# AliBahri94/GM3D

Measured on AMD Instinct MI355X. Metric: point-clouds/sec pretrain step (N=1024,G=64), higher is better.
Workload: dtype bf16

## Files before the change

gm3d_amd/csrc/embed.hip:

```cpp
#include "common.hpp"
#include "guided.hpp"

namespace gm3d {


__device__ __forceinline__ int tpr_of(int C) { return C >> 3; }

__global__ __launch_bounds__(256) void moments3_kernel(const float* __restrict__ x, int R, double* __restrict__ partial) {
    __shared__ double red[4][9];
    double s[9];
#pragma unroll
    for (int i = 0; i < 9; ++i) s[i] = 0.0;
    for (int r = blockIdx.x * 256 + threadIdx.x; r < R; r += gridDim.x * 256) {
        const double a = x[(size_t)r * 3], b = x[(size_t)r * 3 + 1], c = x[(size_t)r * 3 + 2];
        s[0] += a; s[1] += b; s[2] += c;
        s[3] += a * a; s[4] += a * b; s[5] += a * c; s[6] += b * b; s[7] += b * c; s[8] += c * c;
    }
#pragma unroll
    for (int i = 0; i < 9; ++i) {
        double v = s[i];
        for (int o = 32; o > 0; o >>= 1) v += __shfl_xor(v, o);
        if ((threadIdx.x & 63) == 0) red[threadIdx.x >> 6][i] = v;
    }
    __syncthreads();
    if (threadIdx.x < 9) partial[(size_t)blockIdx.x * 9 + threadIdx.x] =
        (red[0][threadIdx.x] + red[1][threadIdx.x]) + (red[2][threadIdx.x] + red[3][threadIdx.x]);
}

template <class T>
__global__ __launch_bounds__(256) void pn_layer1_fwd_kernel(const float* __restrict__ x, const float* __restrict__ wf,
                                                            const float* __restrict__ bf, T* __restrict__ a1, int R, int C1) {
    const int tpr = C1 >> 3;
    const size_t total = (size_t)R * tpr;
    for (size_t t = (size_t)blockIdx.x * 256 + threadIdx.x; t < total; t += (size_t)gridDim.x * 256) {
        const size_t r = t / tpr;
        const int c = (int)(t - r * tpr) * 8;
        const float a = x[r * 3], b = x[r * 3 + 1], d = x[r * 3 + 2];
        float v[8];
#pragma unroll
        for (int i = 0; i < 8; ++i) {
            const float h = a * wf[(c + i) * 3] + b * wf[(c + i) * 3 + 1] + d * wf[(c + i) * 3 + 2] + bf[c + i];
            v[i] = h > 0.f ? h : 0.f;
        }
        V8<T>::store(a1 + r * C1 + c, v);
    }
}

template <class T>
__global__ __launch_bounds__(256) void group_max_fwd_kernel(const T* __restrict__ in, const float* __restrict__ bias,
                                                            T* __restrict__ out, uint8_t* __restrict__ arg, int G, int K, int C) {
    const int tpr = C >> 3, gpb = blockDim.x / tpr;
    const int lane = threadIdx.x % tpr, gl = threadIdx.x / tpr, c = lane * 8;
    for (int g = blockIdx.x * gpb + gl; g < G; g += gridDim.x * gpb) {
        const T* base = in + (size_t)g * K * C + c;
        float best[8];
        int bk[8];
#pragma unroll
        for (int i = 0; i < 8; ++i) { best[i] = -INFINITY; bk[i] = 0; }
        int k = 0;
        for (; k + 8 <= K; k += 8) {
            float v[8][8];
#pragma unroll
            for (int u = 0; u < 8; ++u) V8<T>::load(base + (size_t)(k + u) * C, v[u]);
#pragma unroll
            for (int u = 0; u < 8; ++u)
#pragma unroll
                for (int i = 0; i < 8; ++i)
                    if (v[u][i] > best[i]) { best[i] = v[u][i]; bk[i] = k + u; }
        }
        for (; k < K; ++k) {
            float v[8];
            V8<T>::load(base + (size_t)k * C, v);
#pragma unroll
            for (int i = 0; i < 8; ++i)
                if (v[i] > best[i]) { best[i] = v[i]; bk[i] = k; }
        }
#pragma unroll
        for (int i = 0; i < 8; ++i) {
            if (bias) best[i] += bias[c + i];
            arg[(size_t)g * C + c + i] = (uint8_t)bk[i];
        }
        V8<T>::store(out + (size_t)g * C + c, best);
    }
}

template <class T>
__global__ __launch_bounds__(256) void group_max_bwd_kernel(const T* __restrict__ dout, const uint8_t* __restrict__ arg, T* __restrict__ din,
                                     int G, int K, int C) {
    const int tpr = C >> 3, SL = blockDim.x / tpr;
    const int lane = threadIdx.x % tpr, sl = threadIdx.x / tpr, c = lane * 8;
    for (int g = blockIdx.x; g < G; g += gridDim.x) {
        float d[8];
        V8<T>::load(dout + (size_t)g * C + c, d);
        int a[8];
#pragma unroll
        for (int i = 0; i < 8; ++i) a[i] = arg[(size_t)g * C + c + i];
        for (int k = sl; k < K; k += SL) {
            float v[8];
#pragma unroll
            for (int i = 0; i < 8; ++i) v[i] = a[i] == k ? d[i] : 0.f;
            V8<T>::store(din + ((size_t)g * K + k) * C + c, v);
        }
    }
}

template <int NQ>
__device__ __forceinline__ void write_partials(float (&acc)[NQ][8], float* sm, float* partial, int C, int c, int sl, int SL) {
#pragma unroll
    for (int q = 0; q < NQ; ++q)
#pragma unroll
        for (int i = 0; i < 8; ++i) sm[(size_t)sl * NQ * C + q * C + c + i] = acc[q][i];
    __syncthreads();
    for (int t = threadIdx.x; t < NQ * C; t += blockDim.x) {
        float s = 0.f;
        for (int s2 = 0; s2 < SL; ++s2) s += sm[(size_t)s2 * NQ * C + t];
        partial[(size_t)blockIdx.x * NQ * C + t] = s;
    }
}

template <class T>
__global__ __launch_bounds__(256) void bn_bcast_stats_kernel(const T* __restrict__ y0, const T* __restrict__ t, int G, int K, int C,
                                      float* __restrict__ partial) {
    extern __shared__ float sm[];
    const int tpr = C >> 3, SL = blockDim.x / tpr;
    const int lane = threadIdx.x % tpr, sl = threadIdx.x / tpr, c = lane * 8;
    float acc[2][8];
#pragma unroll
    for (int i = 0; i < 8; ++i) acc[0][i] = acc[1][i] = 0.f;
    for (int g = blockIdx.x; g < G; g += gridDim.x) {
        float tv[8];
        V8<T>::load(t + (size_t)g * C + c, tv);
        for (int k = sl; k < K; k += SL) {
            float v[8];
            V8<T>::load(y0 + ((size_t)g * K + k) * C + c, v);
#pragma unroll
            for (int i = 0; i < 8; ++i) { const float y = v[i] + tv[i]; acc[0][i] += y; acc[1][i] += y * y; }
        }
    }
    write_partials<2>(acc, sm, partial, C, c, sl, SL);
}

template <class T>
__global__ __launch_bounds__(256) void bn_bcast_apply_relu_kernel(const T* __restrict__ y0, const T* __restrict__ t, const float* __restrict__ scale,
                                           const float* __restrict__ shift, T* __restrict__ a2, int G, int K, int C,
                                           float slope, const int* __restrict__ sel ) {
    const int tpr = C >> 3, SL = blockDim.x / tpr;
    const int lane = threadIdx.x % tpr, sl = threadIdx.x / tpr, c = lane * 8;
    float sc[8], sh[8];
#pragma unroll
    for (int i = 0; i < 8; ++i) { sc[i] = scale[c + i]; sh[i] = shift[c + i]; }
    for (int g = blockIdx.x; g < G; g += gridDim.x) {
        const int sg = sel ? sel[g] : g;
        float tv[8];
        V8<T>::load(t + (size_t)sg * C + c, tv);
        for (int k = sl; k < K; k += SL) {
            float v[8];
            V8<T>::load(y0 + ((size_t)sg * K + k) * C + c, v);
#pragma unroll
            for (int i = 0; i < 8; ++i) { const float h = (v[i] + tv[i]) * sc[i] + sh[i]; v[i] = h > 0.f ? h : slope * h; }
            V8<T>::store(a2 + ((size_t)g * K + k) * C + c, v);
        }
    }
}

template <class T>
__global__ __launch_bounds__(256) void bn_bcast_bwd_stats_kernel(const T* __restrict__ da2, const T* __restrict__ y0, const T* __restrict__ t,
                                          const float* __restrict__ scale, const float* __restrict__ shift,
                                          const float* __restrict__ mean, const float* __restrict__ rstd, int G, int K, int C,
                                          float* __restrict__ partial, float slope,
                                          const int* __restrict__ sel ) {
    extern __shared__ float sm[];
    const int tpr = C >> 3, SL = blockDim.x / tpr;
    const int lane = threadIdx.x % tpr, sl = threadIdx.x / tpr, c = lane * 8;
    float sc[8], sh[8], mu[8], rs[8], acc[2][8];
#pragma unroll
    for (int i = 0; i < 8; ++i) { sc[i] = scale[c + i]; sh[i] = shift[c + i]; mu[i] = mean[c + i]; rs[i] = rstd[c + i]; acc[0][i] = acc[1][i] = 0.f; }
    for (int g = blockIdx.x; g < G; g += gridDim.x) {
        const int sg = sel ? sel[g] : g;
        float tv[8];
        V8<T>::load(t + (size_t)sg * C + c, tv);
        for (int k = sl; k < K; k += SL) {
            float v[8], d[8];
            V8<T>::load(y0 + ((size_t)sg * K + k) * C + c, v);
            V8<T>::load(da2 + ((size_t)g * K + k) * C + c, d);
// ... 25 lines not shown
        sc[i] = scale[c + i]; sh[i] = shift[c + i]; mu[i] = mean[c + i]; rs[i] = rstd[c + i];
        m1[i] = s1[c + i] * inv_rows; m2[i] = s2[c + i] * inv_rows;
    }
    for (int g = blockIdx.x * gpb + gl; g < G; g += gridDim.x * gpb) {
        const int cg = inv ? inv[g] : g;
        float tv[8], gs[8];
        V8<T>::load(t + (size_t)g * C + c, tv);
#pragma unroll
        for (int i = 0; i < 8; ++i) gs[i] = 0.f;
        int k = 0;
        for (; k + 4 <= K; k += 4) {
            float v[4][8], d[4][8];
#pragma unroll
            for (int u = 0; u < 4; ++u) {
                V8<T>::load(y0 + ((size_t)g * K + k + u) * C + c, v[u]);
                if (cg >= 0) V8<T>::load(da2 + ((size_t)cg * K + k + u) * C + c, d[u]);
                else {
#pragma unroll
                    for (int i = 0; i < 8; ++i) d[u][i] = 0.f;
                }
            }
#pragma unroll
            for (int u = 0; u < 4; ++u) {
#pragma unroll
                for (int i = 0; i < 8; ++i) {
                    const float y = v[u][i] + tv[i];
                    const float gg = (y * sc[i] + sh[i] > 0.f) ? d[u][i] : slope * d[u][i];
                    const float r = sc[i] * (gg - m1[i] - (y - mu[i]) * rs[i] * m2[i]);
                    v[u][i] = r; gs[i] += r;
                }
                V8<T>::store(dy + ((size_t)g * K + k + u) * C + c, v[u]);
            }
        }
        for (; k < K; ++k) {
            float v[8], d[8] = {0.f, 0.f, 0.f, 0.f, 0.f, 0.f, 0.f, 0.f};
            const size_t o = ((size_t)g * K + k) * C + c;
            V8<T>::load(y0 + o, v);
            if (cg >= 0) V8<T>::load(da2 + ((size_t)cg * K + k) * C + c, d);
#pragma unroll
            for (int i = 0; i < 8; ++i) {
                const float y = v[i] + tv[i];
                const float gg = (y * sc[i] + sh[i] > 0.f) ? d[i] : slope * d[i];
                const float r = sc[i] * (gg - m1[i] - (y - mu[i]) * rs[i] * m2[i]);
                v[i] = r; gs[i] += r;
            }
            V8<T>::store(dy + o, v);
        }
#pragma unroll
        for (int i = 0; i < 8; ++i) dt[(size_t)g * C + c + i] = gs[i];
    }
}

template <class T>
__global__ __launch_bounds__(256) void group_scatter_add_kernel(T* __restrict__ df, const T* __restrict__ dfg, const uint8_t* __restrict__ arg,
                                         int G, int K, int C, float* __restrict__ partial) {
    extern __shared__ float sm[];
    const int tpr = C >> 3, SL = blockDim.x / tpr;
    const int lane = threadIdx.x % tpr, sl = threadIdx.x / tpr, c = lane * 8;
    float acc[1][8];
#pragma unroll
    for (int i = 0; i < 8; ++i) acc[0][i] = 0.f;
    for (int g = blockIdx.x; g < G; g += gridDim.x) {
        float d[8];
        int a[8];
        V8<T>::load(dfg + (size_t)g * C + c, d);
#pragma unroll
        for (int i = 0; i < 8; ++i) a[i] = arg[(size_t)g * C + c + i];
        for (int k = sl; k < K; k += SL) {
            float v[8];
            const size_t o = ((size_t)g * K + k) * C + c;
            V8<T>::load(df + o, v);
            bool hit = false;
#pragma unroll
            for (int i = 0; i < 8; ++i) {
                if (a[i] == k) { v[i] += d[i]; hit = true; }
                acc[0][i] += v[i];
            }
            if (hit) V8<T>::store(df + o, v);
        }
    }
    write_partials<1>(acc, sm, partial, C, c, sl, SL);
}

template <class T>
__global__ __launch_bounds__(256) void pn_layer1_bwd_stats_kernel(const T* __restrict__ da1, const T* __restrict__ a1, const float* __restrict__ x,
                                           const float* __restrict__ w1, const float* __restrict__ b1,
                                           const float* __restrict__ mean, const float* __restrict__ rstd,
                                           const float* __restrict__ xmean, int R, int C1, double* __restrict__ partial) {
    extern __shared__ double smd[];
    const int tpr = C1 >> 3, SL = blockDim.x / tpr;
    const int lane = threadIdx.x % tpr, sl = threadIdx.x / tpr, c = lane * 8;
    float wx[8], wy[8], wz[8], bb[8], rs[8];
    double acc[5][8];
    const float mx = xmean[0], my = xmean[1], mz = xmean[2];
#pragma unroll
    for (int i = 0; i < 8; ++i) {
        wx[i] = w1[(c + i) * 3]; wy[i] = w1[(c + i) * 3 + 1]; wz[i] = w1[(c + i) * 3 + 2];
        bb[i] = b1[c + i] - mean[c + i]; rs[i] = rstd[c + i];
#pragma unroll
        for (int q = 0; q < 5; ++q) acc[q][i] = 0.0;
    }
    for (size_t r = (size_t)blockIdx.x * SL + sl; r < (size_t)R; r += (size_t)gridDim.x * SL) {
        float d[8], a[8];
        V8<T>::load(da1 + r * C1 + c, d);
        V8<T>::load(a1 + r * C1 + c, a);
        const float px = x[r * 3], py = x[r * 3 + 1], pz = x[r * 3 + 2];
#pragma unroll
        for (int i = 0; i < 8; ++i) {
            const float gg = a[i] > 0.f ? d[i] : 0.f;
            const float hh = (px * wx[i] + py * wy[i] + pz * wz[i] + bb[i]) * rs[i];
            acc[0][i] += (double)gg; acc[1][i] += (double)gg * (double)hh;
            acc[2][i] += (double)gg * (double)(px - mx); acc[3][i] += (double)gg * (double)(py - my);
            acc[4][i] += (double)gg * (double)(pz - mz);
        }
    }
#pragma unroll
    for (int q = 0; q < 5; ++q)
#pragma unroll
        for (int i = 0; i < 8; ++i) smd[(size_t)sl * 5 * C1 + q * C1 + c + i] = acc[q][i];
    __syncthreads();
    for (int t = threadIdx.x; t < 5 * C1; t += blockDim.x) {
        double s = 0.0;
        for (int s2 = 0; s2 < SL; ++s2) s += smd[(size_t)s2 * 5 * C1 + t];
        partial[(size_t)blockIdx.x * 5 * C1 + t] = s;
    }
}

template <bool LIN3>
__global__ __launch_bounds__(256) void colsum_finish_f64_kernel(const double* __restrict__ partial, int nrows, int pitch,
                                                                int ncols, double* __restrict__ out, float* __restrict__ dW,
                                                                float* __restrict__ db, int C) {
    __shared__ double red[8][32];
    const int cx = threadIdx.x & 31, slice = threadIdx.x >> 5;
    const int c = blockIdx.x * 32 + cx;
    double s0 = 0.0, s1 = 0.0, s2 = 0.0, s3 = 0.0;
    if (c < ncols) {
        int r = slice;
        for (; r + 24 < nrows; r += 32) {
            s0 += partial[(size_t)r * pitch + c];
            s1 += partial[(size_t)(r + 8) * pitch + c];
            s2 += partial[(size_t)(r + 16) * pitch + c];
            s3 += partial[(size_t)(r + 24) * pitch + c];
        }
        for (; r < nrows; r += 8) s0 += partial[(size_t)r * pitch + c];
    }
    red[slice][cx] = (s0 + s1) + (s2 + s3);
    __syncthreads();
    if (slice == 0 && c < ncols) {
        double t = 0.0;
#pragma unroll
        for (int k = 0; k < 8; ++k) t += red[k][cx];
        if (LIN3) {
            const int which = c / C, cc = c - which * C;
            if (which == 0) db[cc] = (float)t;
            else dW[cc * 3 + which - 1] = (float)t;
        } else {
            out[c] = t;
        }
    }
}

template <class T>
__global__ __launch_bounds__(256) void colsum_partial_kernel(const T* __restrict__ m, int R, int C, float* __restrict__ partial,
                                                             const float* __restrict__ roww) {
    extern __shared__ float sm[];
    const int tpr = C >> 3, SL = blockDim.x / tpr;
    const int lane = threadIdx.x % tpr, sl = threadIdx.x / tpr, c = lane * 8;
    float acc[1][8];
#pragma unroll
    for (int i = 0; i < 8; ++i) acc[0][i] = 0.f;
    for (size_t r = (size_t)blockIdx.x * SL + sl; r < (size_t)R; r += (size_t)gridDim.x * SL) {
        float v[8];
        V8<T>::load(m + r * C + c, v);
        const float wr = roww ? roww[r] : 1.0f;
#pragma unroll
        for (int i = 0; i < 8; ++i) acc[0][i] += wr * v[i];
    }
    write_partials<1>(acc, sm, partial, C, c, sl, SL);
}


__device__ __forceinline__ float gelu3(float x) { return 0.5f * x * (1.0f + erff(x * 0.70710678118654752440f)); }
__device__ __forceinline__ float gelu3_grad(float x) {
    return 0.5f * (1.0f + erff(x * 0.70710678118654752440f)) + x * 0.39894228040143267794f * __expf(-0.5f * x * x);
}

template <class T>
__global__ __launch_bounds__(256) void lin3_gelu_fwd_kernel(const float* __restrict__ x, const float* __restrict__ w,
                                                            const float* __restrict__ b, T* __restrict__ out, int R, int C) {
    const int tpr = C >> 3;
    const size_t total = (size_t)R * tpr;
    for (size_t t = (size_t)blockIdx.x * 256 + threadIdx.x; t < total; t += (size_t)gridDim.x * 256) {
        const size_t r = t / tpr;
        const int c = (int)(t - r * tpr) * 8;
        const float px = x[r * 3], py = x[r * 3 + 1], pz = x[r * 3 + 2];
        float v[8];
#pragma unroll
        for (int i = 0; i < 8; ++i) v[i] = gelu3(px * w[(c + i) * 3] + py * w[(c + i) * 3 + 1] + pz * w[(c + i) * 3 + 2] + b[c + i]);
        V8<T>::store(out + r * C + c, v);
    }
}

template <class T>
__global__ __launch_bounds__(256) void lin3_gelu_bwd_kernel(const T* __restrict__ dout, const float* __restrict__ x, const float* __restrict__ w,
                                     const float* __restrict__ b, int R, int C, double* __restrict__ partial) {
    extern __shared__ double smd[];
    const int tpr = C >> 3, SL = blockDim.x / tpr;
    const int lane = threadIdx.x % tpr, sl = threadIdx.x / tpr, c = lane * 8;
    float wx[8], wy[8], wz[8], bb[8];
    double acc[4][8];
#pragma unroll
    for (int i = 0; i < 8; ++i) {
        wx[i] = w[(c + i) * 3]; wy[i] = w[(c + i) * 3 + 1]; wz[i] = w[(c + i) * 3 + 2]; bb[i] = b[c + i];
#pragma unroll
        for (int q = 0; q < 4; ++q) acc[q][i] = 0.0;
    }
    for (size_t r = (size_t)blockIdx.x * SL + sl; r < (size_t)R; r += (size_t)gridDim.x * SL) {
        float d[8];
        V8<T>::load(dout + r * C + c, d);
        const float px = x[r * 3], py = x[r * 3 + 1], pz = x[r * 3 + 2];
#pragma unroll
        for (int i = 0; i < 8; ++i) {
            const double g = (double)(d[i] * gelu3_grad(px * wx[i] + py * wy[i] + pz * wz[i] + bb[i]));
            acc[0][i] += g; acc[1][i] += g * px; acc[2][i] += g * py; acc[3][i] += g * pz;
        }
    }
#pragma unroll
    for (int q = 0; q < 4; ++q)
#pragma unroll
        for (int i = 0; i < 8; ++i) smd[(size_t)sl * 4 * C + q * C + c + i] = acc[q][i];
    __syncthreads();
    for (int t = threadIdx.x; t < 4 * C; t += blockDim.x) {
        double s = 0.0;
        for (int s2 = 0; s2 < SL; ++s2) s += smd[(size_t)s2 * 4 * C + t];
        partial[(size_t)blockIdx.x * 4 * C + t] = s;
    }
}

__global__ __launch_bounds__(64) void rank_loss_kernel(const float* __restrict__ p, int ldp, const float* __restrict__ t, int M,
                                                       float* __restrict__ out, float* __restrict__ dp) {
    const int b = blockIdx.x, j = threadIdx.x;
    const float pj = j < M ? p[(size_t)b * ldp + j] : 0.f, tj = j < M ? t[(size_t)b * M + j] : 0.f;
    float ls = 0.f, cnt = 0.f, g = 0.f;
    for (int i = 0; i < M; ++i) {
        const float pi = __shfl(pj, i), ti = __shfl(tj, i);
        if (j < M) {
            const float sg = 1.0f / (1.0f + __expf(-(pj - pi)));
            const float ds = sg * (1.0f - sg);
            if (tj > ti) { ls -= __logf(sg + 1e-6f); cnt += 1.f; g -= ds / (sg + 1e-6f); }
            else if (tj < ti) { ls -= __logf(1.0f - sg + 1e-6f); cnt += 1.f; g += ds / (1.0f - sg + 1e-6f); }
            const float s2 = 1.0f / (1.0f + __expf(-(pi - pj)));
            const float d2 = s2 * (1.0f - s2);
            if (ti > tj) g += d2 / (s2 + 1e-6f);
            else if (ti < tj) g -= d2 / (1.0f - s2 + 1e-6f);
        }
    }
    for (int o = 32; o > 0; o >>= 1) { ls += __shfl_xor(ls, o); cnt += __shfl_xor(cnt, o); }
    if (j == 0) { out[(size_t)b * 2] = ls; out[(size_t)b * 2 + 1] = cnt; }
    if (j < M) dp[(size_t)b * M + j] = g;
}

__global__ __launch_bounds__(256) void rank_loss_finish_kernel(const float* __restrict__ out, int B, float* __restrict__ tot,
                                                               float* __restrict__ loss) {
    __shared__ float red[2][256];
    float a = 0.f, c = 0.f;
    for (int b = threadIdx.x; b < B; b += 256) { a += out[(size_t)b * 2]; c += out[(size_t)b * 2 + 1]; }
    red[0][threadIdx.x] = a; red[1][threadIdx.x] = c;
    __syncthreads();
    for (int o = 128; o > 0; o >>= 1) {
        if ((int)threadIdx.x < o) { red[0][threadIdx.x] += red[0][threadIdx.x + o]; red[1][threadIdx.x] += red[1][threadIdx.x + o]; }
        __syncthreads();
    }
    if (threadIdx.x == 0) { tot[0] = red[0][0]; tot[1] = red[1][0]; loss[0] = red[0][0] / red[1][0]; }
}

__global__ __launch_bounds__(256) void rank_loss_bwd_kernel(const float* __restrict__ dp, const float* __restrict__ g,
                                                            const float* __restrict__ tot, int B, int M, int L, float* __restrict__ dfull) {
    const int i = blockIdx.x * 256 + threadIdx.x;
    if (i >= B * L) return;
    const int b = i / L, l = i - b * L, j = l - (L - M);
    const float s = g[0] / tot[1];
    dfull[i] = j >= 0 ? dp[(size_t)b * M + j] * s : 0.f;
}

__global__ void ema_counters_kernel(long long* __restrict__ e, const long long* __restrict__ m, int n, float decay, float w) {
#pragma clang fp contract(off)
    const int i = blockIdx.x * blockDim.x + threadIdx.x;
    if (i < n) {
        const float a = (float)e[i] * decay, b = w * (float)m[i];
        e[i] = (long long)(a + b);
    }
}

__global__ __launch_bounds__(256) void drop_path_scales_kernel(const float* __restrict__ u, const float* __restrict__ keep, int S, int B,
                                                               float* __restrict__ out) {
    const int i = blockIdx.x * 256 + threadIdx.x;
    if (i >= S * B) return;
    const float k = keep[i / B];
    out[i] = __fdiv_rn(floorf(__fadd_rn(u[i], k)), k);
}

template <class T>
__global__ __launch_bounds__(256) void pad_cols_kernel(const T* __restrict__ src, size_t lds, int R, int N, T* __restrict__ dst, int Np) {
    const int cpr = Np >> 3;
    const size_t i = (size_t)blockIdx.x * 256 + threadIdx.x;
    if (i >= (size_t)R * cpr) return;
    const size_t r = i / cpr;
    const int c = (int)(i - r * cpr) * 8;
    float v[8];
#pragma unroll
    for (int e = 0; e < 8; ++e) v[e] = 0.f;
    if (c < N) V8<T>::load(src + r * lds + c, v);
    V8<T>::store(dst + r * (size_t)Np + c, v);
}

__global__ void bn_finalize_kernel(const float* __restrict__ sums , double rows,
                                   const float* __restrict__ gamma, const float* __restrict__ beta, float eps, float momentum,
                                   float* __restrict__ running_mean, float* __restrict__ running_var,
                                   long long* __restrict__ nbt, float* __restrict__ scale, float* __restrict__ shift,
                                   float* __restrict__ mean_out, float* __restrict__ rstd_out, int C, int training) {
    const int c = blockIdx.x * blockDim.x + threadIdx.x;
    if (c == 0 && training && nbt) nbt[0] += 1;
    if (c >= C) return;
    double mean, var;
    if (training) {
        mean = (double)sums[c] / rows;
        var = (double)sums[C + c] / rows - mean * mean;
        if (var < 0.0) var = 0.0;
        running_mean[c] = (float)((1.0 - momentum) * running_mean[c] + momentum * mean);
        running_var[c] = (float)((1.0 - momentum) * running_var[c] + momentum * var * (rows / (rows - 1.0)));
    } else {
        mean = running_mean[c]; var = running_var[c];
    }
    const double rstd = 1.0 / sqrt(var + (double)eps);
    const double sc = (double)gamma[c] * rstd;
    scale[c] = (float)sc;
    shift[c] = (float)((double)beta[c] - mean * sc);
    mean_out[c] = (float)mean;
    rstd_out[c] = (float)rstd;
}

__global__ void pn1_finalize_kernel(const double* __restrict__ mom9, double rows, const float* __restrict__ w ,
// ... 219 lines not shown
    }
}

template <class T>
__global__ __launch_bounds__(64) void token_assemble_fwd_kernel(const T* __restrict__ tokens, const T* __restrict__ pos,
                                                                const long long* __restrict__ order, int L, int V, int C,
                                                                T* __restrict__ x_vis, T* __restrict__ pos_vis,
                                                                T* __restrict__ pos_full) {
    const int b = blockIdx.x / L, j = blockIdx.x - b * L;
    const int i = (int)order[(size_t)b * L + j];
    const size_t src = ((size_t)b * L + i) * C, dfull = ((size_t)b * L + j) * C, dvis = ((size_t)b * V + j) * C;
    for (int c = threadIdx.x * 8; c < C; c += 64 * 8) {
        float p[8];
        V8<T>::load(pos + src + c, p);
        V8<T>::store(pos_full + dfull + c, p);
        if (j < V) {
            V8<T>::store(pos_vis + dvis + c, p);
            if (tokens) {
                float t[8];
                V8<T>::load(tokens + src + c, t);
                V8<T>::store(x_vis + dvis + c, t);
            }
        }
    }
}

template <class T>
__global__ __launch_bounds__(64) void token_assemble_bwd_kernel(const T* __restrict__ dx_vis, const T* __restrict__ dpos_vis,
                                                                const T* __restrict__ dpos_full, const long long* __restrict__ order,
                                                                int L, int V, int C, T* __restrict__ dtokens, T* __restrict__ dpos) {
    const int b = blockIdx.x / L, j = blockIdx.x - b * L;
    const int i = (int)order[(size_t)b * L + j];
    const size_t dst = ((size_t)b * L + i) * C, sfull = ((size_t)b * L + j) * C, svis = ((size_t)b * V + j) * C;
    for (int c = threadIdx.x * 8; c < C; c += 64 * 8) {
        float g[8] = {0.f, 0.f, 0.f, 0.f, 0.f, 0.f, 0.f, 0.f}, t[8] = {0.f, 0.f, 0.f, 0.f, 0.f, 0.f, 0.f, 0.f};
        if (dpos_full) V8<T>::load(dpos_full + sfull + c, g);
        if (j < V) {
            if (dpos_vis) {
                float v[8];
                V8<T>::load(dpos_vis + svis + c, v);
#pragma unroll
                for (int e = 0; e < 8; ++e) g[e] += v[e];
            }
            if (dx_vis) V8<T>::load(dx_vis + svis + c, t);
        }
        V8<T>::store(dpos + dst + c, g);
        if (dtokens) V8<T>::store(dtokens + dst + c, t);
    }
}

static inline bool chan_ok(int C) { return C >= 8 && C % 8 == 0 && C <= 1024; }
static inline int threads_for(int C) { const int tpr = C / 8; int sl = 256 / tpr; if (sl < 1) sl = 1; return sl * tpr; }
static inline int slices_for(int C) { const int tpr = C / 8; int sl = 256 / tpr; return sl < 1 ? 1 : sl; }
static inline int group_grid(int G) { return G < 1024 ? G : 1024; }
static inline int row_grid(int R, int C) { const int sl = slices_for(C); int g = (R + sl - 1) / sl; return g < 1 ? 1 : (g > 1024 ? 1024 : g); }
static inline int moments_grid(int R) { int g = (R + 255) / 256; return g < 1 ? 1 : (g > 256 ? 256 : g); }
static inline int pn1_slices(int C1) { return C1 > 200 ? 4 : 8; }
static inline int lin3_slices(int C) { return C > 256 ? 4 : 8; }
static inline int slice_grid(int R, int sl) { int g = (R + sl - 1) / sl; return g > 1024 ? 1024 : (g < 1 ? 1 : g); }

}

extern "C" int gm3d_embed_partial_rows(int kind, int n, int C) {
    using namespace gm3d;
    if (kind == 0) return moments_grid(n);
    if (kind == 1) return group_grid(n);
    if (kind == 3) return slice_grid(n, lin3_slices(C));
    if (kind == 4) return slice_grid(n, pn1_slices(C));
    return row_grid(n, C);
}

extern "C" int gm3d_moments3(const float* x, int R, double* partial, gm3d_stream_t stream) {
    using namespace gm3d;
    if (!x || !partial || R < 1) return GM3D_EINVAL;
    return launch_lds<moments3_kernel>(dim3(moments_grid(R)), dim3(256), 0, stream, x, R, partial);
}

extern "C" int gm3d_pn_layer1_fwd(const float* x, const float* wf, const float* bf, void* a1, int R, int C1, int dtype,
                                  gm3d_stream_t stream) {
    using namespace gm3d;
    if (!x || !wf || !bf || !a1 || R < 1) return GM3D_EINVAL;
    if (!chan_ok(C1)) return GM3D_EUNSUPPORTED;
    if (dtype != GM3D_F32 && dtype != GM3D_BF16) return GM3D_EINVAL;
    const size_t total = (size_t)R * (C1 / 8);
    const int grid = (int)((total + 255) / 256 < 4096 ? (total + 255) / 256 : 4096);
    return by_dtype(dtype, [&](auto* t) {
        using T = std::remove_pointer_t<decltype(t)>;
        return launch_lds<pn_layer1_fwd_kernel<T>>(dim3(grid), dim3(256), 0, stream, x, wf, bf, (T*)a1, R, C1);
    });
}

static int gkc_check(const void* a, const void* b, int G, int K, int C, int dtype) {
    if (!a || !b || G < 1 || K < 1) return GM3D_EINVAL;
    if (!gm3d::chan_ok(C) || K > 255) return GM3D_EUNSUPPORTED;
    if (dtype != GM3D_F32 && dtype != GM3D_BF16) return GM3D_EINVAL;
    return GM3D_OK;
}

extern "C" int gm3d_group_max_fwd(const void* in, const float* bias, void* out, uint8_t* arg, int G, int K, int C, int dtype,
                                  gm3d_stream_t stream) {
    using namespace gm3d;
    int rc = gkc_check(in, out, G, K, C, dtype);
    if (rc != GM3D_OK) return rc;
    if (!arg) return GM3D_EINVAL;
    const int gpb = 256 / (C / 8) < 1 ? 1 : 256 / (C / 8);
    int grid = (G + gpb - 1) / gpb; grid = grid > 8192 ? 8192 : grid;
    return by_dtype(dtype, [&](auto* t) {
        using T = std::remove_pointer_t<decltype(t)>;
        return launch_lds<group_max_fwd_kernel<T>>(dim3(grid), dim3(gpb * (C / 8)), 0, stream,
                                                   (const T*)in, bias, (T*)out, arg, G, K, C);
    });
}

extern "C" int gm3d_group_max_bwd(const void* dout, const uint8_t* arg, void* din, int G, int K, int C, int dtype,
                                  gm3d_stream_t stream) {
    using namespace gm3d;
    int rc = gkc_check(dout, din, G, K, C, dtype);
    if (rc != GM3D_OK) return rc;
    if (!arg) return GM3D_EINVAL;
    return by_dtype(dtype, [&](auto* t) {
        using T = std::remove_pointer_t<decltype(t)>;
        return launch_lds<group_max_bwd_kernel<T>>(dim3(group_grid(G)), dim3(threads_for(C)), 0, stream,
                                                   (const T*)dout, arg, (T*)din, G, K, C);
    });
}

extern "C" int gm3d_bn_bcast_stats(const void* y0, const void* t, int G, int K, int C, float* partial, int dtype,
                                   gm3d_stream_t stream) {
    using namespace gm3d;
    int rc = gkc_check(y0, t, G, K, C, dtype);
    if (rc != GM3D_OK) return rc;
    if (!partial) return GM3D_EINVAL;
    const size_t lds = (size_t)slices_for(C) * 2 * C * 4;
    return by_dtype(dtype, [&](auto* e) {
        using T = std::remove_pointer_t<decltype(e)>;
        return launch_lds<bn_bcast_stats_kernel<T>>(dim3(group_grid(G)), dim3(threads_for(C)), lds, stream,
                                                    (const T*)y0, (const T*)t, G, K, C, partial);
    });
}

extern "C" int gm3d_bn_bcast_apply_relu_sel(const void* y0, const void* t, const float* scale, const float* shift, void* a2,
                                            const int* sel, int G, int K, int C, float slope, int dtype, gm3d_stream_t stream) {
    using namespace gm3d;
    int rc = gkc_check(y0, t, G, K, C, dtype);
    if (rc != GM3D_OK) return rc;
    if (!scale || !shift || !a2) return GM3D_EINVAL;
    return by_dtype(dtype, [&](auto* e) {
        using T = std::remove_pointer_t<decltype(e)>;
        return launch_lds<bn_bcast_apply_relu_kernel<T>>(dim3(group_grid(G)), dim3(threads_for(C)), 0, stream,
                                                         (const T*)y0, (const T*)t, scale, shift, (T*)a2, G, K, C, slope, sel);
    });
}

extern "C" int gm3d_bn_bcast_apply_relu(const void* y0, const void* t, const float* scale, const float* shift, void* a2,
                                        int G, int K, int C, float slope, int dtype, gm3d_stream_t stream) {
    return gm3d_bn_bcast_apply_relu_sel(y0, t, scale, shift, a2, nullptr, G, K, C, slope, dtype, stream);
}

extern "C" int gm3d_bn_bcast_bwd_stats_sel(const void* da2, const void* y0, const void* t, const float* scale,
                                           const float* shift, const float* mean, const float* rstd, const int* sel, int G, int K,
                                           int C, float* partial, float slope, int dtype, gm3d_stream_t stream) {
    using namespace gm3d;
    int rc = gkc_check(y0, t, G, K, C, dtype);
    if (rc != GM3D_OK) return rc;
    if (!da2 || !scale || !shift || !mean || !rstd || !partial) return GM3D_EINVAL;
    const size_t lds = (size_t)slices_for(C) * 2 * C * 4;
    return by_dtype(dtype, [&](auto* e) {
        using T = std::remove_pointer_t<decltype(e)>;
        return launch_lds<bn_bcast_bwd_stats_kernel<T>>(dim3(group_grid(G)), dim3(threads_for(C)), lds, stream, (const T*)da2,
                                                        (const T*)y0, (const T*)t, scale, shift, mean, rstd, G, K, C, partial, slope, sel);
    });
}

extern "C" int gm3d_bn_bcast_bwd_stats(const void* da2, const void* y0, const void* t, const float* scale,
                                       const float* shift, const float* mean, const float* rstd, int G, int K, int C,
                                       float* partial, float slope, int dtype, gm3d_stream_t stream) {
    return gm3d_bn_bcast_bwd_stats_sel(da2, y0, t, scale, shift, mean, rstd, nullptr, G, K, C, partial, slope, dtype, stream);
}

extern "C" int gm3d_bn_bcast_bwd_apply_sel(const void* da2, const void* y0, const void* t, const float* scale,
                                           const float* shift, const float* mean, const float* rstd, const float* s1,
                                           const float* s2, void* dy, float* dt, const int* inv, int G, int K, int C, float slope,
                                           int dtype, gm3d_stream_t stream) {
    using namespace gm3d;
    int rc = gkc_check(y0, t, G, K, C, dtype);
    if (rc != GM3D_OK) return rc;
    if (!da2 || !scale || !shift || !mean || !rstd || !s1 || !s2 || !dy || !dt) return GM3D_EINVAL;
    const float inv_rows = 1.0f / ((float)G * (float)K);
    const int gpb = 256 / (C / 8) < 1 ? 1 : 256 / (C / 8);
    int grid = (G + gpb - 1) / gpb; grid = grid > 8192 ? 8192 : grid;
    return by_dtype(dtype, [&](auto* e) {
        using T = std::remove_pointer_t<decltype(e)>;
        return launch_lds<bn_bcast_bwd_apply_kernel<T>>(dim3(grid), dim3(gpb * (C / 8)), 0, stream,
                                                        (const T*)da2, (const T*)y0, (const T*)t, scale, shift, mean, rstd, s1, s2,
                                                        inv_rows, (T*)dy, dt, G, K, C, slope, inv);
    });
}

extern "C" int gm3d_bn_bcast_bwd_apply(const void* da2, const void* y0, const void* t, const float* scale,
                                       const float* shift, const float* mean, const float* rstd, const float* s1,
                                       const float* s2, void* dy, float* dt, int G, int K, int C, float slope, int dtype,
                                       gm3d_stream_t stream) {
    return gm3d_bn_bcast_bwd_apply_sel(da2, y0, t, scale, shift, mean, rstd, s1, s2, dy, dt, nullptr, G, K, C, slope, dtype, stream);
}

// ... 83 lines not shown
                                        double* partial, int dtype, gm3d_stream_t stream) {
    using namespace gm3d;
    if (!da1 || !a1 || !x || !w1 || !b1 || !mean || !rstd || !xmean || !partial || R < 1) return GM3D_EINVAL;
    if (!chan_ok(C1) || C1 > 256) return GM3D_EUNSUPPORTED;
    if (dtype != GM3D_F32 && dtype != GM3D_BF16) return GM3D_EINVAL;
    const int tpr = C1 / 8, sl = pn1_slices(C1);
    const size_t lds = (size_t)sl * 5 * C1 * sizeof(double);
    const int grid = slice_grid(R, sl);
    return by_dtype(dtype, [&](auto* t) {
        using T = std::remove_pointer_t<decltype(t)>;
        return launch_lds<pn_layer1_bwd_stats_kernel<T>>(dim3(grid), dim3(sl * tpr), lds, stream,
                                                         (const T*)da1, (const T*)a1, x, w1, b1, mean, rstd, xmean, R, C1, partial);
    });
}

extern "C" int gm3d_colsum_finish_f64(const double* partial, int nrows, int pitch, int ncols, double* out,
                                      gm3d_stream_t stream) {
    using namespace gm3d;
    if (!partial || !out || nrows < 0 || ncols < 1 || pitch < ncols) return GM3D_EINVAL;
    return launch_lds<colsum_finish_f64_kernel<false>>(dim3((ncols + 31) / 32), dim3(256), 0, stream, partial, nrows, pitch, ncols, out,
                                                       nullptr, nullptr, 1);
}

extern "C" int gm3d_lin3_finish(const double* partial, int nrows, int C, float* dW, float* db, gm3d_stream_t stream) {
    using namespace gm3d;
    if (!partial || !dW || !db || nrows < 0 || C < 1) return GM3D_EINVAL;
    return launch_lds<colsum_finish_f64_kernel<true>>(dim3((4 * C + 31) / 32), dim3(256), 0, stream, partial, nrows, 4 * C, 4 * C,
                                                      nullptr, dW, db, C);
}

extern "C" int gm3d_colsum_partial_w(const void* m, const float* roww, int R, int C, float* partial, int dtype, gm3d_stream_t stream);
extern "C" int gm3d_colsum_partial(const void* m, int R, int C, float* partial, int dtype, gm3d_stream_t stream) {
    return gm3d_colsum_partial_w(m, nullptr, R, C, partial, dtype, stream);
}

extern "C" int gm3d_colsum_partial_w(const void* m, const float* roww, int R, int C, float* partial, int dtype, gm3d_stream_t stream) {
    using namespace gm3d;
    if (!m || !partial || R < 1) return GM3D_EINVAL;
    if (C < 8 || C % 8 || C > 2048) return GM3D_EUNSUPPORTED;
    if (dtype != GM3D_F32 && dtype != GM3D_BF16) return GM3D_EINVAL;
    const size_t lds = (size_t)slices_for(C) * C * 4;
    return by_dtype(dtype, [&](auto* t) {
        using T = std::remove_pointer_t<decltype(t)>;
        return launch_lds<colsum_partial_kernel<T>>(dim3(row_grid(R, C)), dim3(threads_for(C)), lds, stream,
                                                    (const T*)m, R, C, partial, roww);
    });
}

extern "C" int gm3d_lin3_gelu_fwd(const float* x, const float* w, const float* b, void* out, int R, int C, int dtype,
                                  gm3d_stream_t stream) {
    using namespace gm3d;
    if (!x || !w || !b || !out || R < 1) return GM3D_EINVAL;
    if (!chan_ok(C)) return GM3D_EUNSUPPORTED;
    if (dtype != GM3D_F32 && dtype != GM3D_BF16) return GM3D_EINVAL;
    const size_t total = (size_t)R * (C / 8);
    const int grid = (int)((total + 255) / 256 < 4096 ? (total + 255) / 256 : 4096);
    return by_dtype(dtype, [&](auto* t) {
        using T = std::remove_pointer_t<decltype(t)>;
        return launch_lds<lin3_gelu_fwd_kernel<T>>(dim3(grid), dim3(256), 0, stream, x, w, b, (T*)out, R, C);
    });
}

extern "C" int gm3d_lin3_gelu_bwd(const void* dout, const float* x, const float* w, const float* b, int R, int C,
                                  double* partial, int dtype, gm3d_stream_t stream) {
    using namespace gm3d;
    if (!dout || !x || !w || !b || !partial || R < 1) return GM3D_EINVAL;
    if (!chan_ok(C) || C > 512) return GM3D_EUNSUPPORTED;
    if (dtype != GM3D_F32 && dtype != GM3D_BF16) return GM3D_EINVAL;
    const int tpr = C / 8, sl = lin3_slices(C);
    const size_t lds = (size_t)sl * 4 * C * sizeof(double);
    const int grid = slice_grid(R, sl);
    return by_dtype(dtype, [&](auto* t) {
        using T = std::remove_pointer_t<decltype(t)>;
        return launch_lds<lin3_gelu_bwd_kernel<T>>(dim3(grid), dim3(sl * tpr), lds, stream, (const T*)dout, x, w, b, R, C, partial);
    });
}

extern "C" int gm3d_rank_loss(const float* pred, const float* target, int B, int M, float* out, float* dpred,
                              gm3d_stream_t stream) {
    using namespace gm3d;
    if (!pred || !target || !out || !dpred || B < 1 || M < 1) return GM3D_EINVAL;
    if (M > GUIDED_MAX) return GM3D_EUNSUPPORTED;
    if (M > GUIDED_NARROW) return launch_rank_loss_wide(pred, M, target, B, M, out, dpred, stream);
    return launch_lds<rank_loss_kernel>(dim3(B), dim3(64), 0, stream, pred, M, target, M, out, dpred);
}

extern "C" int gm3d_rank_loss_tail(const float* pred, int ldp, const float* target, int B, int M, float* out, float* dpred, float* tot,
                                   float* loss, gm3d_stream_t stream) {
    using namespace gm3d;
    if (!pred || !target || !out || !dpred || !tot || !loss || B < 1 || M < 1 || ldp < M) return GM3D_EINVAL;
    if (M > GUIDED_MAX) return GM3D_EUNSUPPORTED;
    const int rc = M > GUIDED_NARROW ? launch_rank_loss_wide(pred, ldp, target, B, M, out, dpred, stream)
                                     : launch_lds<rank_loss_kernel>(dim3(B), dim3(64), 0, stream, pred, ldp, target, M, out, dpred);
    if (rc != GM3D_OK) return rc;
    return launch_lds<rank_loss_finish_kernel>(dim3(1), dim3(256), 0, stream, (const float*)out, B, tot, loss);
}

extern "C" int gm3d_rank_loss_tail_bwd(const float* dpred, const float* g, const float* tot, int B, int M, int L, float* dfull,
                                       gm3d_stream_t stream) {
    using namespace gm3d;
    if (!dpred || !g || !tot || !dfull || B < 1 || M < 1 || L < M) return GM3D_EINVAL;
    return launch_lds<rank_loss_bwd_kernel>(dim3((B * L + 255) / 256), dim3(256), 0, stream, dpred, g, tot, B, M, L, dfull);
}

extern "C" int gm3d_ema_counters(long long* e, const long long* m, int n, float decay, float w, gm3d_stream_t stream) {
    using namespace gm3d;
    if (!e || !m || n < 0) return GM3D_EINVAL;
    if (n == 0) return GM3D_OK;
    return launch_lds<ema_counters_kernel>(dim3((n + 63) / 64), dim3(64), 0, stream, e, m, n, decay, w);
}

extern "C" int gm3d_drop_path_scales(const float* u, const float* keep, int S, int B, float* out, gm3d_stream_t stream) {
    using namespace gm3d;
    if (!u || !keep || !out || S < 1 || B < 1) return GM3D_EINVAL;
    return launch_lds<drop_path_scales_kernel>(dim3((S * B + 255) / 256), dim3(256), 0, stream, u, keep, S, B, out);
}

extern "C" int gm3d_pad_cols(const void* src, long long lds, int R, int N, void* dst, int Np, int dtype, gm3d_stream_t stream) {
    using namespace gm3d;
    if (!src || !dst || R < 1 || N < 1 || Np < N || lds < N) return GM3D_EINVAL;
    if (N % 8 || Np % 8 || lds % 8) return GM3D_EUNSUPPORTED;
    if (dtype != GM3D_F32 && dtype != GM3D_BF16) return GM3D_EINVAL;
    const size_t n = (size_t)R * (Np / 8);
    return by_dtype(dtype, [&](auto* t) {
        using T = std::remove_pointer_t<decltype(t)>;
        return launch_lds<pad_cols_kernel<T>>(dim3((unsigned)((n + 255) / 256)), dim3(256), 0, stream, (const T*)src, (size_t)lds, R, N,
                                              (T*)dst, Np);
    });
}

extern "C" int gm3d_bn_finalize(const float* sums, double rows, const float* gamma, const float* beta, float eps,
                                float momentum, float* running_mean, float* running_var, long long* nbt, float* scale,
                                float* shift, float* mean_out, float* rstd_out, int C, int training, gm3d_stream_t stream) {
    using namespace gm3d;
    if (!gamma || !beta || !running_mean || !running_var || !scale || !shift || !mean_out || !rstd_out || C < 1) return GM3D_EINVAL;
    if (training && (!sums || rows < 2.0)) return GM3D_EINVAL;
    return launch_lds<bn_finalize_kernel>(dim3((C + 255) / 256), dim3(256), 0, stream, sums, rows, gamma, beta, eps, momentum,
                                          running_mean, running_var, nbt, scale, shift, mean_out, rstd_out, C, training);
}

extern "C" int gm3d_pn1_finalize(const double* mom9, double rows, const float* w, const float* b, const float* gamma,
                                 const float* beta, float eps, float momentum, float* running_mean, float* running_var,
                                 long long* nbt, float* wf, float* bf, float* mean_out, float* rstd_out, double* mcov,
                                 float* xmean, int C, int training, gm3d_stream_t stream) {
    using namespace gm3d;
    if (!w || !b || !gamma || !beta || !running_mean || !running_var || !wf || !bf || !mean_out || !rstd_out || C < 1) return GM3D_EINVAL;
    if (training && (!mom9 || rows < 2.0)) return GM3D_EINVAL;
    return launch_lds<pn1_finalize_kernel>(dim3((C + 255) / 256), dim3(256), 0, stream, mom9, rows, w, b, gamma, beta, eps, momentum,
                                           running_mean, running_var, nbt, wf, bf, mean_out, rstd_out, mcov, xmean, C, training);
}

extern "C" int gm3d_pn1_bwd_finalize(const double* q, const double* mcov, const float* w, const float* gamma, const float* rstd,
                                     float* dw, float* dgamma, float* dbeta, int C, gm3d_stream_t stream) {
    using namespace gm3d;
    if (!q || !mcov || !w || !gamma || !rstd || !dw || !dgamma || !dbeta || C < 1) return GM3D_EINVAL;
    return launch_lds<pn1_bwd_finalize_kernel>(dim3((C + 255) / 256), dim3(256), 0, stream, q, mcov, w, gamma, rstd, dw, dgamma, dbeta, C);
}

extern "C" int gm3d_mask_select_b(const float* loss_pred, const float* noise, int B, int L, int len_keep, int len_loss, float* mask,
                                  unsigned char* mask_bool, long long* vis_ids, long long* mask_ids, int id_pitch, gm3d_stream_t stream);

extern "C" int gm3d_mask_select(const float* loss_pred, const float* noise, int B, int L, int len_keep, int len_loss,
                                float* mask, long long* vis_ids, long long* mask_ids, int id_pitch, gm3d_stream_t stream) {
    return gm3d_mask_select_b(loss_pred, noise, B, L, len_keep, len_loss, mask, nullptr, vis_ids, mask_ids, id_pitch, stream);
}

extern "C" int gm3d_mask_select_b(const float* loss_pred, const float* noise, int B, int L, int len_keep, int len_loss, float* mask,
                                  unsigned char* mask_bool, long long* vis_ids, long long* mask_ids, int id_pitch, gm3d_stream_t stream) {
    using namespace gm3d;
    if (!loss_pred || !noise || !mask || !vis_ids || !mask_ids || B < 0 || L < 1) return GM3D_EINVAL;
    if (len_keep < 0 || len_loss < 0 || len_keep + len_loss > L) return GM3D_EINVAL;
    if (L > GUIDED_MAX) return GM3D_EUNSUPPORTED;
    if (B == 0) return GM3D_OK;
    if (id_pitch != 0 && id_pitch < L) return GM3D_EINVAL;
    if (L > GUIDED_NARROW)
        return launch_mask_select_wide(loss_pred, noise, B, L, len_keep, len_loss, mask, mask_bool, vis_ids, mask_ids,
// ... 34 lines not shown
```

Before: 17020.

## Rework several embed kernels: register-cached weights, software-pipelined bwd stats, split rank loss

The layer-1 forward kernel now gives each thread a fixed channel slice and keeps its weights in registers, replacing a per-element division and repeated weight loads. The group-max backward kernel assigns one group per thread slice, loads the 8 argmax bytes in a single 64-bit read, and writes rows sequentially. The layer-1 backward stats kernel double-buffers its row loads with sched barriers and hints two blocks per SM to hide memory latency. The rank-loss kernel spreads the pairwise loop over four wavefronts and reduces through LDS. These are separate, unrelated edits; the new alignment check on arg and the larger LDS use in rank loss add constraints and overhead.

```diff
diff --git a/gm3d_amd/csrc/embed.hip b/gm3d_amd/csrc/embed.hip
--- a/gm3d_amd/csrc/embed.hip
+++ b/gm3d_amd/csrc/embed.hip
@@ -30,16 +30,18 @@
 template <class T>
 __global__ __launch_bounds__(256) void pn_layer1_fwd_kernel(const float* __restrict__ x, const float* __restrict__ wf,
                                                             const float* __restrict__ bf, T* __restrict__ a1, int R, int C1) {
-    const int tpr = C1 >> 3;
-    const size_t total = (size_t)R * tpr;
-    for (size_t t = (size_t)blockIdx.x * 256 + threadIdx.x; t < total; t += (size_t)gridDim.x * 256) {
-        const size_t r = t / tpr;
-        const int c = (int)(t - r * tpr) * 8;
+    const int tpr = C1 >> 3, SL = blockDim.x / tpr;
+    const int lane = threadIdx.x % tpr, sl = threadIdx.x / tpr, c = lane * 8;
+    float wx[8], wy[8], wz[8], bb[8];
+#pragma unroll
+    for (int i = 0; i < 8; ++i) { wx[i] = wf[(c + i) * 3]; wy[i] = wf[(c + i) * 3 + 1]; wz[i] = wf[(c + i) * 3 + 2]; bb[i] = bf[c + i]; }
+    const int step = gridDim.x * SL;
+    for (long long r = blockIdx.x * SL + sl; r < R; r += step) {
         const float a = x[r * 3], b = x[r * 3 + 1], d = x[r * 3 + 2];
         float v[8];
 #pragma unroll
         for (int i = 0; i < 8; ++i) {
-            const float h = a * wf[(c + i) * 3] + b * wf[(c + i) * 3 + 1] + d * wf[(c + i) * 3 + 2] + bf[c + i];
+            const float h = a * wx[i] + b * wy[i] + d * wz[i] + bb[i];
             v[i] = h > 0.f ? h : 0.f;
         }
         V8<T>::store(a1 + r * C1 + c, v);
@@ -87,19 +89,21 @@
 template <class T>
 __global__ __launch_bounds__(256) void group_max_bwd_kernel(const T* __restrict__ dout, const uint8_t* __restrict__ arg, T* __restrict__ din,
                                      int G, int K, int C) {
-    const int tpr = C >> 3, SL = blockDim.x / tpr;
-    const int lane = threadIdx.x % tpr, sl = threadIdx.x / tpr, c = lane * 8;
-    for (int g = blockIdx.x; g < G; g += gridDim.x) {
+    const int tpr = C >> 3, gpb = blockDim.x / tpr;
+    const int lane = threadIdx.x % tpr, gl = threadIdx.x / tpr, c = lane * 8;
+    for (int g = blockIdx.x * gpb + gl; g < G; g += gridDim.x * gpb) {
         float d[8];
         V8<T>::load(dout + (size_t)g * C + c, d);
+        const unsigned long long w = *reinterpret_cast<const unsigned long long*>(arg + (size_t)g * C + c);
         int a[8];
 #pragma unroll
-        for (int i = 0; i < 8; ++i) a[i] = arg[(size_t)g * C + c + i];
-        for (int k = sl; k < K; k += SL) {
+        for (int i = 0; i < 8; ++i) a[i] = (int)((w >> (8 * i)) & 0xffull);
+        T* row = din + (size_t)g * K * C + c;
+        for (int k = 0; k < K; ++k) {
             float v[8];
 #pragma unroll
             for (int i = 0; i < 8; ++i) v[i] = a[i] == k ? d[i] : 0.f;
-            V8<T>::store(din + ((size_t)g * K + k) * C + c, v);
+            V8<T>::store(row + (size_t)k * C, v);
         }
     }
 }
@@ -291,11 +295,27 @@
     write_partials<1>(acc, sm, partial, C, c, sl, SL);
 }
 
-template <class T>
-__global__ __launch_bounds__(256) void pn_layer1_bwd_stats_kernel(const T* __restrict__ da1, const T* __restrict__ a1, const float* __restrict__ x,
+template <class T> struct Raw8;
+template <> struct Raw8<float> {
+    float4 lo, hi;
+    __device__ __forceinline__ void ld(const float* p) { lo = *reinterpret_cast<const float4*>(p); hi = *reinterpret_cast<const float4*>(p + 4); }
+    __device__ __forceinline__ void get(float* v) const { v[0] = lo.x; v[1] = lo.y; v[2] = lo.z; v[3] = lo.w; v[4] = hi.x; v[5] = hi.y; v[6] = hi.z; v[7] = hi.w; }
+};
+template <> struct Raw8<bf16_t> {
+    V8<bf16_t>::v8 q;
+    __device__ __forceinline__ void ld(const bf16_t* p) { q = *reinterpret_cast<const V8<bf16_t>::v8*>(p); }
+    __device__ __forceinline__ void get(float* v) const {
+#pragma unroll
+        for (int i = 0; i < 8; ++i) v[i] = (float)q[i];
+    }
+};
+
+template <class T>
+__global__ __launch_bounds__(256, 2) void pn_layer1_bwd_stats_kernel(const T* __restrict__ da1, const T* __restrict__ a1, const float* __restrict__ x,
                                            const float* __restrict__ w1, const float* __restrict__ b1,
                                            const float* __restrict__ mean, const float* __restrict__ rstd,
                                            const float* __restrict__ xmean, int R, int C1, double* __restrict__ partial) {
+    using R8 = Raw8<T>;
     extern __shared__ double smd[];
     const int tpr = C1 >> 3, SL = blockDim.x / tpr;
     const int lane = threadIdx.x % tpr, sl = threadIdx.x / tpr, c = lane * 8;
@@ -309,11 +329,9 @@
 #pragma unroll
         for (int q = 0; q < 5; ++q) acc[q][i] = 0.0;
     }
-    for (size_t r = (size_t)blockIdx.x * SL + sl; r < (size_t)R; r += (size_t)gridDim.x * SL) {
+    auto add_row = [&](const R8& dr, const R8& ar, float px, float py, float pz) {
         float d[8], a[8];
-        V8<T>::load(da1 + r * C1 + c, d);
-        V8<T>::load(a1 + r * C1 + c, a);
-        const float px = x[r * 3], py = x[r * 3 + 1], pz = x[r * 3 + 2];
+        dr.get(d); ar.get(a);
 #pragma unroll
         for (int i = 0; i < 8; ++i) {
             const float gg = a[i] > 0.f ? d[i] : 0.f;
@@ -322,6 +340,47 @@
             acc[2][i] += (double)gg * (double)(px - mx); acc[3][i] += (double)gg * (double)(py - my);
             acc[4][i] += (double)gg * (double)(pz - mz);
         }
+    };
+    const size_t step = (size_t)gridDim.x * SL, sC = step * C1, s3 = step * 3;
+    size_t r = (size_t)blockIdx.x * SL + sl;
+    const T* pd = da1 + r * C1 + c;
+    const T* pa = a1 + r * C1 + c;
+    const float* pp = x + r * 3;
+    constexpr int PF = 4 / (int)sizeof(T);
+    struct Batch { R8 d[PF], a[PF]; float px[PF], py[PF], pz[PF]; };
+    auto load = [&](Batch& b, size_t ahead) {
+#pragma unroll
+        for (int u = 0; u < PF; ++u) {
+            const size_t o = ahead * PF + u;
+            b.d[u].ld(pd + o * sC); b.a[u].ld(pa + o * sC);
+            b.px[u] = pp[o * s3]; b.py[u] = pp[o * s3 + 1]; b.pz[u] = pp[o * s3 + 2];
+        }
+    };
+    auto add = [&](const Batch& b) {
+#pragma unroll
+        for (int u = 0; u < PF; ++u) {
+            __builtin_amdgcn_sched_barrier(0);
+            add_row(b.d[u], b.a[u], b.px[u], b.py[u], b.pz[u]);
+        }
+        r += PF * step; pd += PF * sC; pa += PF * sC; pp += PF * s3;
+    };
+    auto whole = [&](size_t ahead) { return r + ((ahead + 1) * PF - 1) * step < (size_t)R; };
+    Batch q0, q1;
+    if (whole(0)) load(q0, 0);
+    while (whole(0)) {
+        const bool n1 = whole(1);
+        if (n1) load(q1, 1);
+        add(q0);
+        if (!n1) break;
+        const bool n0 = whole(1);
+        if (n0) load(q0, 1);
+        add(q1);
+        if (!n0) break;
+    }
+    for (; r < (size_t)R; r += step, pd += sC, pa += sC, pp += s3) {
+        R8 d, a;
+        d.ld(pd); a.ld(pa);
+        add_row(d, a, pp[0], pp[1], pp[2]);
     }
 #pragma unroll
     for (int q = 0; q < 5; ++q)
@@ -446,27 +505,41 @@
     }
 }
 
-__global__ __launch_bounds__(64) void rank_loss_kernel(const float* __restrict__ p, int ldp, const float* __restrict__ t, int M,
-                                                       float* __restrict__ out, float* __restrict__ dp) {
-    const int b = blockIdx.x, j = threadIdx.x;
+__global__ __launch_bounds__(256) void rank_loss_kernel(const float* __restrict__ p, int ldp, const float* __restrict__ t, int M,
+                                                        float* __restrict__ out, float* __restrict__ dp) {
+    __shared__ float term[3][64][64];
+    __shared__ float cw[4][64];
+    const int b = blockIdx.x, j = threadIdx.x & 63, w = threadIdx.x >> 6;
     const float pj = j < M ? p[(size_t)b * ldp + j] : 0.f, tj = j < M ? t[(size_t)b * M + j] : 0.f;
-    float ls = 0.f, cnt = 0.f, g = 0.f;
-    for (int i = 0; i < M; ++i) {
+    float cnt = 0.f;
+    for (int i = w; i < M; i += 4) {
         const float pi = __shfl(pj, i), ti = __shfl(tj, i);
+        float l = 0.f, a = 0.f, c = 0.f;
         if (j < M) {
             const float sg = 1.0f / (1.0f + __expf(-(pj - pi)));
             const float ds = sg * (1.0f - sg);
-            if (tj > ti) { ls -= __logf(sg + 1e-6f); cnt += 1.f; g -= ds / (sg + 1e-6f); }
-            else if (tj < ti) { ls -= __logf(1.0f - sg + 1e-6f); cnt += 1.f; g += ds / (1.0f - sg + 1e-6f); }
+            if (tj > ti) { l = -__logf(sg + 1e-6f); cnt += 1.f; a = -(ds / (sg + 1e-6f)); }
+            else if (tj < ti) { l = -__logf(1.0f - sg + 1e-6f); cnt += 1.f; a = ds / (1.0f - sg + 1e-6f); }
             const float s2 = 1.0f / (1.0f + __expf(-(pi - pj)));
             const float d2 = s2 * (1.0f - s2);
-            if (ti > tj) g += d2 / (s2 + 1e-6f);
-            else if (ti < tj) g -= d2 / (1.0f - s2 + 1e-6f);
-        }
-    }
-    for (int o = 32; o > 0; o >>= 1) { ls += __shfl_xor(ls, o); cnt += __shfl_xor(cnt, o); }
-    if (j == 0) { out[(size_t)b * 2] = ls; out[(size_t)b * 2 + 1] = cnt; }
-    if (j < M) dp[(size_t)b * M + j] = g;
+            if (ti > tj) c = d2 / (s2 + 1e-6f);
+            else if (ti < tj) c = -(d2 / (1.0f - s2 + 1e-6f));
+        }
+        term[0][i][j] = l; term[1][i][j] = a; term[2][i][j] = c;
+    }
+    cw[w][j] = cnt;
+    __syncthreads();
+    if (w == 0) {
+        float ls = 0.f;
+        for (int i = 0; i < M; ++i) ls += term[0][i][j];
+        cnt = (cw[0][j] + cw[1][j]) + (cw[2][j] + cw[3][j]);
+        for (int o = 32; o > 0; o >>= 1) { ls += __shfl_xor(ls, o); cnt += __shfl_xor(cnt, o); }
+        if (j == 0) { out[(size_t)b * 2] = ls; out[(size_t)b * 2 + 1] = cnt; }
+    } else if (w == 1) {
+        float g = 0.f;
+        for (int i = 0; i < M; ++i) { g += term[1][i][j]; g += term[2][i][j]; }
+        if (j < M) dp[(size_t)b * M + j] = g;
+    }
 }
 
 __global__ __launch_bounds__(256) void rank_loss_finish_kernel(const float* __restrict__ out, int B, float* __restrict__ tot,
@@ -852,11 +925,12 @@
     if (!x || !wf || !bf || !a1 || R < 1) return GM3D_EINVAL;
     if (!chan_ok(C1)) return GM3D_EUNSUPPORTED;
     if (dtype != GM3D_F32 && dtype != GM3D_BF16) return GM3D_EINVAL;
-    const size_t total = (size_t)R * (C1 / 8);
-    const int grid = (int)((total + 255) / 256 < 4096 ? (total + 255) / 256 : 4096);
+    const int sl = slices_for(C1);
+    const long long want = ((long long)R + sl - 1) / sl;
+    const int grid = want > 2048 ? 2048 : (int)want;
     return by_dtype(dtype, [&](auto* t) {
         using T = std::remove_pointer_t<decltype(t)>;
-        return launch_lds<pn_layer1_fwd_kernel<T>>(dim3(grid), dim3(256), 0, stream, x, wf, bf, (T*)a1, R, C1);
+        return launch_lds<pn_layer1_fwd_kernel<T>>(dim3(grid), dim3(threads_for(C1)), 0, stream, x, wf, bf, (T*)a1, R, C1);
     });
 }
 
@@ -887,10 +961,13 @@
     using namespace gm3d;
     int rc = gkc_check(dout, din, G, K, C, dtype);
     if (rc != GM3D_OK) return rc;
-    if (!arg) return GM3D_EINVAL;
+    if (!arg || ((uintptr_t)arg & 7)) return GM3D_EINVAL;
+    const int gpb = slices_for(C);
+    const long long want = ((long long)G + gpb - 1) / gpb;
+    const int grid = want > 2048 ? 2048 : (int)want;
     return by_dtype(dtype, [&](auto* t) {
         using T = std::remove_pointer_t<decltype(t)>;
-        return launch_lds<group_max_bwd_kernel<T>>(dim3(group_grid(G)), dim3(threads_for(C)), 0, stream,
+        return launch_lds<group_max_bwd_kernel<T>>(dim3(grid), dim3(threads_for(C)), 0, stream,
                                                    (const T*)dout, arg, (T*)din, G, K, C);
     });
 }
@@ -1140,7 +1217,7 @@
     if (!pred || !target || !out || !dpred || B < 1 || M < 1) return GM3D_EINVAL;
     if (M > GUIDED_MAX) return GM3D_EUNSUPPORTED;
     if (M > GUIDED_NARROW) return launch_rank_loss_wide(pred, M, target, B, M, out, dpred, stream);
-    return launch_lds<rank_loss_kernel>(dim3(B), dim3(64), 0, stream, pred, M, target, M, out, dpred);
+    return launch_lds<rank_loss_kernel>(dim3(B), dim3(256), 0, stream, pred, M, target, M, out, dpred);
 }
 
 extern "C" int gm3d_rank_loss_tail(const float* pred, int ldp, const float* target, int B, int M, float* out, float* dpred, float* tot,
@@ -1149,7 +1226,7 @@
     if (!pred || !target || !out || !dpred || !tot || !loss || B < 1 || M < 1 || ldp < M) return GM3D_EINVAL;
     if (M > GUIDED_MAX) return GM3D_EUNSUPPORTED;
     const int rc = M > GUIDED_NARROW ? launch_rank_loss_wide(pred, ldp, target, B, M, out, dpred, stream)
-                                     : launch_lds<rank_loss_kernel>(dim3(B), dim3(64), 0, stream, pred, ldp, target, M, out, dpred);
+                                     : launch_lds<rank_loss_kernel>(dim3(B), dim3(256), 0, stream, pred, ldp, target, M, out, dpred);
     if (rc != GM3D_OK) return rc;
     return launch_lds<rank_loss_finish_kernel>(dim3(1), dim3(256), 0, stream, (const float*)out, B, tot, loss);
 }
```

Result: no change. 17150 (median of 6 runs) (+0.8%).
